# apache/arrow-rs

Measured on NVIDIA B200. Metric: Mrows/sec filter+take+add on 1e9-row Int64/Float64; % HBM roofline, higher is better.
Workload: dtype i64 (filter/take/sum) + f64 (add)

## Files before the change

arrow-rs_b200/csrc/compact.cu:

```cuda
#include <cstdlib>
#include <vector>

#include "bitmap.cuh"
#include "internal.cuh"

#define TILE_ROWS 1024
#define TILE_WORDS (TILE_ROWS / 64)
#define SCAN_CHUNK 4096

struct acu_filter_plan {
  int64_t len = 0;
  int64_t count = 0;
  int32_t strategy = ACU_FILTER_NONE;
  int64_t n_tiles = 0;
  uint64_t *mask = nullptr;
  uint64_t *tile_off = nullptr;
  uint32_t *tile_count = nullptr;
  uint64_t *chunk_total = nullptr;
  void *storage = nullptr;
  mutable void *index_cache = nullptr;
};

namespace {

__global__ void __launch_bounds__(256) k_plan_mask(const uint8_t *__restrict__ pv, int64_t poff,
                                                   const uint8_t *__restrict__ nv, int64_t noff,
                                                   int64_t len, int64_t n_words_padded, uint64_t *__restrict__ mask,
                                                   uint32_t *__restrict__ tile_count, int64_t n_tiles) {
  const int lane = threadIdx.x & 31;
  const int64_t warp = ((int64_t)blockIdx.x * blockDim.x + threadIdx.x) >> 5;
  const int64_t nwarps = ((int64_t)gridDim.x * blockDim.x) >> 5;
  for (int64_t w0 = warp * 32; w0 < n_words_padded; w0 += nwarps * 32) {
    const int64_t w = w0 + lane;
    const int64_t row = w << 6;
    uint64_t m = ld_bits64(pv, poff + row, poff + len);
    if (nv) m &= ld_bits64(nv, noff + row, noff + len);
    mask[w] = m;
    unsigned c = __popcll(m);
#pragma unroll
    for (int o = 8; o > 0; o >>= 1) c += __shfl_xor_sync(ACU_FULL_MASK, c, o);
    const int64_t t = w >> 4;
    if ((lane & 15) == 0 && t < n_tiles) tile_count[t] = c;
  }
}

__global__ void __launch_bounds__(1024) k_plan_scan_chunks(const uint32_t *__restrict__ tile_count, int64_t n_tiles,
                                                           uint64_t *__restrict__ tile_off,
                                                           uint64_t *__restrict__ chunk_total) {
  __shared__ uint32_t warp_tot[32];
  const int64_t base = (int64_t)blockIdx.x * SCAN_CHUNK + (int64_t)threadIdx.x * 4;
  uint32_t c[4];
#pragma unroll
  for (int k = 0; k < 4; ++k) c[k] = (base + k < n_tiles) ? tile_count[base + k] : 0u;
  uint32_t mine = c[0] + c[1] + c[2] + c[3];
  uint32_t incl = mine;
  const int lane = threadIdx.x & 31, wid = threadIdx.x >> 5;
#pragma unroll
  for (int o = 1; o < 32; o <<= 1) {
    uint32_t y = __shfl_up_sync(ACU_FULL_MASK, incl, o);
    if (lane >= o) incl += y;
  }
  if (lane == 31) warp_tot[wid] = incl;
  __syncthreads();
  if (wid == 0) {
    uint32_t w = warp_tot[lane], wi = w;
#pragma unroll
    for (int o = 1; o < 32; o <<= 1) {
      uint32_t y = __shfl_up_sync(ACU_FULL_MASK, wi, o);
      if (lane >= o) wi += y;
    }
    warp_tot[lane] = wi - w;
    if (lane == 31) chunk_total[blockIdx.x] = wi;
  }
  __syncthreads();
  uint32_t excl = warp_tot[wid] + incl - mine;
#pragma unroll
  for (int k = 0; k < 4; ++k) {
    if (base + k < n_tiles) tile_off[base + k] = excl;
    excl += c[k];
  }
}

__global__ void __launch_bounds__(1024) k_plan_scan_top(uint64_t *__restrict__ chunk_total, int64_t n_chunks,
                                                        unsigned long long *__restrict__ res) {
  __shared__ uint64_t warp_tot[32];
  __shared__ uint64_t carry_s;
  if (threadIdx.x == 0) carry_s = 0;
  __syncthreads();
  const int lane = threadIdx.x & 31, wid = threadIdx.x >> 5;
  for (int64_t base = 0; base < n_chunks; base += 1024) {
    const int64_t i = base + threadIdx.x;
    uint64_t v = i < n_chunks ? chunk_total[i] : 0ull, incl = v;
#pragma unroll
    for (int o = 1; o < 32; o <<= 1) {
      uint64_t y = __shfl_up_sync(ACU_FULL_MASK, incl, o);
      if (lane >= o) incl += y;
    }
    if (lane == 31) warp_tot[wid] = incl;
    __syncthreads();
    if (wid == 0) {
      uint64_t w = warp_tot[lane], wi = w;
#pragma unroll
      for (int o = 1; o < 32; o <<= 1) {
        uint64_t y = __shfl_up_sync(ACU_FULL_MASK, wi, o);
        if (lane >= o) wi += y;
      }
      warp_tot[lane] = wi - w;
    }
    __syncthreads();
    const uint64_t carry = carry_s;
    if (i < n_chunks) chunk_total[i] = carry + warp_tot[wid] + incl - v;
    __syncthreads();
    if (threadIdx.x == 1023) carry_s = carry + warp_tot[31] + incl;
    __syncthreads();
  }
  if (threadIdx.x == 0) res[RES_COUNT] = carry_s;
}

__global__ void __launch_bounds__(256) k_plan_finalize(uint64_t *__restrict__ tile_off, int64_t n_tiles, int64_t n_padded,
                                                       const uint64_t *__restrict__ chunk_off,
                                                       const unsigned long long *__restrict__ res) {
  const int64_t stride = (int64_t)gridDim.x * blockDim.x;
  for (int64_t t = (int64_t)blockIdx.x * blockDim.x + threadIdx.x; t < n_padded; t += stride)
    tile_off[t] = t < n_tiles ? tile_off[t] + chunk_off[t / SCAN_CHUNK] : res[RES_COUNT];
}

struct FilterArgs {
  const uint8_t *values;
  uint8_t *out;
  const uint64_t *mask;
  const uint64_t *tile_off;
  int64_t n_tiles;
  int aligned16;
  const uint8_t *vsrc;
  int64_t voff;
  int64_t vlen;
  uint32_t *vout;
  unsigned long long *res;
};

constexpr int BATCH_COLS = 8;
struct FilterBatch { FilterArgs col[BATCH_COLS]; };

template <int W>
__global__ void __launch_bounds__(256, 4) k_filter_values(const FilterBatch batch) {
  const FilterArgs &a = batch.col[blockIdx.y];
  constexpr int CPT = TILE_ROWS * W / 16;
  constexpr int ITERS = CPT / 32;
  constexpr int BATCH = ITERS < 8 ? ITERS : 8;
  constexpr int RPC = W <= 16 ? 16 / W : 1;
  constexpr int CPR = W <= 16 ? 1 : W / 16;
  const int lane = threadIdx.x & 31;
  const int64_t warp = ((int64_t)blockIdx.x * blockDim.x + threadIdx.x) >> 5;
  const int64_t nwarps = ((int64_t)gridDim.x * blockDim.x) >> 5;

  int64_t t = warp;
  uint64_t m_next = 0, off_next = 0, end_next = 0;
  if (t < a.n_tiles) {
    if (lane < TILE_WORDS) m_next = __ldg(a.mask + t * TILE_WORDS + lane);
    off_next = __ldg(a.tile_off + t);
    end_next = __ldg(a.tile_off + t + 1);
  }
  for (; t < a.n_tiles; t += nwarps) {
    const uint64_t m = m_next, out0 = off_next, cnt = end_next - off_next;
    const int64_t tn = t + nwarps;
    if (tn < a.n_tiles) {
      m_next = (lane < TILE_WORDS) ? __ldg(a.mask + tn * TILE_WORDS + lane) : 0ull;
      off_next = __ldg(a.tile_off + tn);
      end_next = __ldg(a.tile_off + tn + 1);
    }
    if (cnt == 0) continue;
    const uint32_t c = __popcll(m);
    uint32_t incl = c;
#pragma unroll
    for (int o = 1; o < TILE_WORDS; o <<= 1) {
      uint32_t y = __shfl_up_sync(ACU_FULL_MASK, incl, o);
      if (lane >= o) incl += y;
    }
    const uint32_t pref = incl - c;
    const uint8_t *src = a.values + (size_t)t * TILE_ROWS * W;
    uint8_t *dst = a.out + (size_t)out0 * W;
#pragma unroll 1
    for (int b0 = 0; b0 < ITERS; b0 += BATCH) {
      uint4 v[BATCH];
      uint32_t bits[BATCH];
      uint32_t rank[BATCH];
#pragma unroll
      for (int j = 0; j < BATCH; ++j) {
        const int cidx = (b0 + j) * 32 + lane;
        const int r = cidx * RPC / CPR;
        const uint64_t word = __shfl_sync(ACU_FULL_MASK, m, r >> 6);
        const uint32_t wp = __shfl_sync(ACU_FULL_MASK, pref, r >> 6);
        bits[j] = (uint32_t)(word >> (r & 63)) & ((1u << RPC) - 1u);
        rank[j] = wp + __popcll(word & ((1ull << (r & 63)) - 1ull));
        if (bits[j]) {
          if (a.aligned16) {
            v[j] = ld_stream16(src + (size_t)cidx * 16);
          } else {
            if constexpr (W >= 8) {
              const uint64_t *p = reinterpret_cast<const uint64_t *>(src + (size_t)cidx * 16);
              const uint64_t lo = (W > 8 || (bits[j] & 1u)) ? __ldg(p) : 0ull;
              const uint64_t hi = (W > 8 || (bits[j] & 2u)) ? __ldg(p + 1) : 0ull;
              v[j] = make_uint4((uint32_t)lo, (uint32_t)(lo >> 32), (uint32_t)hi, (uint32_t)(hi >> 32));
            } else if constexpr (W == 4) {
              const uint32_t *p = reinterpret_cast<const uint32_t *>(src + (size_t)cidx * 16);
              v[j].x = (bits[j] & 1u) ? __ldg(p) : 0u;
              v[j].y = (bits[j] & 2u) ? __ldg(p + 1) : 0u;
              v[j].z = (bits[j] & 4u) ? __ldg(p + 2) : 0u;
              v[j].w = (bits[j] & 8u) ? __ldg(p + 3) : 0u;
            } else {
              uint8_t *vb = reinterpret_cast<uint8_t *>(&v[j]);
              const uint8_t *p = src + (size_t)cidx * 16;
#pragma unroll
              for (int e = 0; e < 16; ++e) vb[e] = ((bits[j] >> (e / W)) & 1u) ? __ldg(p + e) : (uint8_t)0;
// ... 224 lines not shown
    __syncwarp();
    const uint8_t *src = a.values + (size_t)t * TILE_ROWS * W;
    uint8_t *dst = a.out + (size_t)out0 * W;
#pragma unroll 1
    for (int pass = 0; pass < C::PASSES; ++pass) {
      const int half_base = (pass * C::PASS_ROWS) >> 5;
      const uint8_t *psrc = src + ((size_t)pass * C::CPP + lane) * 16;
      asm volatile("" : "+l"(psrc));
      const uint32_t *hh = &s_h[wid][half_base + lr_half];
      uint32_t sel = 0;
#pragma unroll
      for (int j = 0; j < C::ITERS; ++j) {
        const int r0 = j * RPJ;
        const uint32_t bits = (hh[r0 >> 5] >> ((r0 & 31) + lr_bit)) & F::CHUNK_MASK;
        sel |= bits << (j * RPC);
        if (bits) cp_async16(lbuf + j * 32, psrc + (size_t)j * 512);
      }
      cp_async_wait_all();
      __syncwarp();
      const uint32_t *hp = &s_hp[wid][half_base + lr_half];
#pragma unroll
      for (int j = 0; j < C::ITERS; ++j) {
        const uint32_t bits = (sel >> (j * RPC)) & F::CHUNK_MASK;
        const int r0 = j * RPJ;
        const int sh = (r0 & 31) + lr_bit;
        const uint32_t rank = hp[r0 >> 5] + __popc(hh[r0 >> 5] & ((1u << sh) - 1u));
        const uint4 x = lbuf[j * 32];
        if constexpr (W == 8) {
          uint64_t *o = reinterpret_cast<uint64_t *>(dst) + rank;
          if (bits & 1u) o[0] = (uint64_t)x.x | ((uint64_t)x.y << 32);
          if (bits & 2u) o[bits & 1u] = (uint64_t)x.z | ((uint64_t)x.w << 32);
        } else if constexpr (W == 4) {
          uint32_t *o = reinterpret_cast<uint32_t *>(dst) + rank;
          if (bits & 1u) *o++ = x.x;
          if (bits & 2u) *o++ = x.y;
          if (bits & 4u) *o++ = x.z;
          if (bits & 8u) *o = x.w;
        } else if constexpr (W == 2) {
          uint16_t *o = reinterpret_cast<uint16_t *>(dst) + rank;
          const uint16_t *ve = reinterpret_cast<const uint16_t *>(&x);
#pragma unroll
          for (int e = 0; e < 8; ++e)
            if ((bits >> e) & 1u) *o++ = ve[e];
        } else if constexpr (W == 1) {
          uint8_t *o = dst + rank;
          const uint8_t *ve = reinterpret_cast<const uint8_t *>(&x);
#pragma unroll
          for (int e = 0; e < 16; ++e)
            if ((bits >> e) & 1u) *o++ = ve[e];
        } else {
          if (bits) {
            const int half = lane % CPR;
            uint64_t *o = reinterpret_cast<uint64_t *>(dst + (size_t)rank * W + half * 16);
            o[0] = (uint64_t)x.x | ((uint64_t)x.y << 32);
            o[1] = (uint64_t)x.z | ((uint64_t)x.w << 32);
          }
        }
      }
      __syncwarp();
    }
    if (vsrc) {
      const uint32_t c = __popcll(m);
      if (c) {
        const uint64_t bits = pext64_sparse(v, m, c);
        valid_cnt += __popcll(bits);
        const uint64_t p = out0 + s_hp[wid][(2 * lane) & 31];
        const uint32_t sh = (uint32_t)p & 31u;
        uint32_t *o = a.vout + (p >> 5);
        const uint32_t w0 = (uint32_t)(bits << sh);
        const uint64_t rest = sh ? (bits >> (32u - sh)) : (bits >> 32);
        if (w0) atomicOr(o, w0);
        if ((uint32_t)rest) atomicOr(o + 1, (uint32_t)rest);
        if ((uint32_t)(rest >> 32)) atomicOr(o + 2, (uint32_t)(rest >> 32));
      }
      __syncwarp();
    }
  }
  if (vsrc && a.res) {
    valid_cnt = warp_sum(valid_cnt);
    if (lane == 0 && valid_cnt) atomicAdd(a.res + RES_COUNT, (unsigned long long)valid_cnt);
  }
}

struct CompressArgs {
  const uint8_t *src;
  int64_t soff;
  uint32_t *out;
  unsigned long long *res;
  uint64_t out_bytes;
  const uint64_t *count_ptr;
};
struct CompressBatch { CompressArgs col[BATCH_COLS]; };

__global__ void __launch_bounds__(256) k_zero_outputs(const CompressBatch batch) {
  const CompressArgs &c = batch.col[blockIdx.y];
  uint64_t *o = reinterpret_cast<uint64_t *>(c.out);
  const uint64_t words = c.count_ptr ? ((*c.count_ptr + 63) >> 6) : (c.out_bytes >> 3);
  for (uint64_t i = (uint64_t)blockIdx.x * blockDim.x + threadIdx.x; i < words; i += (uint64_t)gridDim.x * blockDim.x) o[i] = 0ull;
}
__global__ void __launch_bounds__(256) k_zero_bitmap_dev(uint64_t *__restrict__ o, const uint64_t *__restrict__ count_ptr) {
  const uint64_t words = (*count_ptr + 63) >> 6;
  for (uint64_t i = (uint64_t)blockIdx.x * blockDim.x + threadIdx.x; i < words; i += (uint64_t)gridDim.x * blockDim.x) o[i] = 0ull;
}

__global__ void __launch_bounds__(256, 8) k_compress_bits(const CompressBatch batch, int64_t len, const uint64_t *__restrict__ mask,
                                                       const uint64_t *__restrict__ tile_off, int64_t n_words_padded) {
  const uint8_t *__restrict__ src = batch.col[blockIdx.y].src;
  const int64_t soff = batch.col[blockIdx.y].soff;
  uint32_t *__restrict__ out = batch.col[blockIdx.y].out;
  unsigned long long *__restrict__ res = batch.col[blockIdx.y].res;
  __shared__ uint32_t s_win[8][68];
  const int lane = threadIdx.x & 31, wid = threadIdx.x >> 5;
  const int64_t warp = ((int64_t)blockIdx.x * blockDim.x + threadIdx.x) >> 5;
  const int64_t nwarps = ((int64_t)gridDim.x * blockDim.x) >> 5;
  unsigned valid_cnt = 0;
  for (int64_t w0 = warp * 32; w0 < n_words_padded; w0 += nwarps * 32) {
    const int64_t w = w0 + lane;
    uint64_t m = __ldg(mask + w);
    const uint32_t cnt = __popcll(m);
    uint32_t incl = cnt;
#pragma unroll
    for (int o = 1; o < 32; o <<= 1) {
      uint32_t y = __shfl_up_sync(ACU_FULL_MASK, incl, o);
      if (lane >= o) incl += y;
    }
    const uint32_t total = __shfl_sync(ACU_FULL_MASK, incl, 31);
    if (total == 0) continue;
    const uint64_t base = __ldg(tile_off + (w0 >> 4));
    uint64_t bits = 0;
    if (m) {
      const uint64_t v = ld_bits64(src, soff + (w << 6), soff + len);
      const uint64_t ones = m & v, zeros = m & ~v;
      const bool clear_mode = __popcll(zeros) <= __popcll(ones);
      uint64_t it = clear_mode ? zeros : ones, acc = 0;
      while (it) {
        const int b = __ffsll((long long)it) - 1;
        it &= it - 1;
        acc |= 1ull << __popcll(m & ((1ull << b) - 1ull));
      }
      const uint64_t full = cnt == 64 ? ~0ull : ((1ull << cnt) - 1ull);
      bits = clear_mode ? (full & ~acc) : acc;
    }
    valid_cnt += __popcll(bits);
    const uint32_t lead = (uint32_t)(base & 31);
    const uint32_t nwords = (lead + total + 31) >> 5;
    for (uint32_t i = lane; i < nwords; i += 32) s_win[wid][i] = 0;
    __syncwarp();
    if (cnt) {
      const uint32_t p = lead + incl - cnt;
      const uint32_t sh = p & 31;
      atomicOr(&s_win[wid][p >> 5], (uint32_t)(bits << sh));
      if (sh + cnt > 32) {
        const uint64_t rest = bits >> (32 - sh);
        atomicOr(&s_win[wid][(p >> 5) + 1], (uint32_t)rest);
        if (sh + cnt > 64) atomicOr(&s_win[wid][(p >> 5) + 2], (uint32_t)(rest >> 32));
      }
    }
    __syncwarp();
    uint32_t *o = out + (base >> 5);
    for (uint32_t i = lane; i < nwords; i += 32) {
      const uint32_t word = s_win[wid][i];
      if (i == 0 || i == nwords - 1) { if (word) atomicOr(o + i, word); }
      else o[i] = word;
    }
    __syncwarp();
  }
  if (res) {
    valid_cnt = warp_sum(valid_cnt);
    if (lane == 0 && valid_cnt) atomicAdd(res + RES_COUNT, (unsigned long long)valid_cnt);
  }
}

acu_status check_len(acu_ctx *ctx, const acu_filter_plan *plan, int64_t values_len) {
  if (plan->len > values_len)
    return acu_fail(ctx, ACU_ERR_INVALID_ARGUMENT, -1, 0, 0, (uint64_t)values_len,
                    "Filter predicate of length %lld is larger than target array of length %lld",
                    (long long)plan->len, (long long)values_len);
  return ACU_OK;
}

template <int W>
acu_status launch_filter(acu_ctx *ctx, const FilterBatch &fb, int n_cols, bool fused) {
  const FilterArgs &fa = fb.col[0];
  if (fa.aligned16) {
    if (!fused) {
      constexpr size_t smem = 8 * (size_t)AsyncCfg<W>::PASS_BYTES;
      if (ctx->occupancy.find(reinterpret_cast<const void *>(k_filter_values_async<W>)) == ctx->occupancy.end())
        ACU_CUDA(ctx, cudaFuncSetAttribute(k_filter_values_async<W>, cudaFuncAttributeMaxDynamicSharedMemorySize, (int)smem));
      const int gx = acu_wave_grid(ctx, k_filter_values_async<W>, 256, smem, (fa.n_tiles + 7) / 8);
      ACU_LAUNCH_TIMED(ctx, ACU_K_FILTER, (k_filter_values_async<W>), dim3(gx, n_cols), 256, smem, fb);
      return ACU_OK;
    }
    constexpr size_t smem = 8 * (size_t)AsyncCfg<W>::PASS_BYTES;
    if (ctx->occupancy.find(reinterpret_cast<const void *>(k_filter_fused<W>)) == ctx->occupancy.end())
      ACU_CUDA(ctx, cudaFuncSetAttribute(k_filter_fused<W>, cudaFuncAttributeMaxDynamicSharedMemorySize, (int)smem));
    static const int tiles_per_warp = getenv("ACU_FILTER_TILES_PER_WARP") ? atoi(getenv("ACU_FILTER_TILES_PER_WARP")) : 4;
    const int64_t want = (fa.n_tiles + 8 * (int64_t)tiles_per_warp - 1) / (8 * (int64_t)tiles_per_warp);
    int gx = acu_wave_grid(ctx, k_filter_fused<W>, 256, smem, (fa.n_tiles + 7) / 8);
    gx = (gx + n_cols - 1) / n_cols;
    if (gx > want) gx = (int)(want < 1 ? 1 : want);
    ACU_LAUNCH_TIMED(ctx, ACU_K_FILTER, (k_filter_fused<W>), dim3(gx, n_cols), 256, smem, fb);
  } else {
    const int gx = acu_wave_grid(ctx, k_filter_values<W>, 256, 0, (fa.n_tiles + 7) / 8);
    ACU_LAUNCH_TIMED(ctx, ACU_K_FILTER, (k_filter_values<W>), dim3(gx, n_cols), 256, 0, fb);
  }
  return ACU_OK;
}

acu_status launch_filter_width(acu_ctx *ctx, int32_t elem_bytes, const FilterBatch &fb, int n_cols, bool fused) {
  switch (elem_bytes) {
    case 1: return launch_filter<1>(ctx, fb, n_cols, fused);
    case 2: return launch_filter<2>(ctx, fb, n_cols, fused);
    case 4: return launch_filter<4>(ctx, fb, n_cols, fused);
    case 8: return launch_filter<8>(ctx, fb, n_cols, fused);
    case 16: return launch_filter<16>(ctx, fb, n_cols, fused);
    case 32: return launch_filter<32>(ctx, fb, n_cols, fused);
    default:
      return acu_fail(ctx, ACU_ERR_INVALID_ARGUMENT, -1, 0, 0, 0, "filter: unsupported element width %d", elem_bytes);
  }
}

acu_status launch_compress(acu_ctx *ctx, const acu_filter_plan *plan, const CompressBatch &cb, int n_cols) {
  const int64_t n_words_padded = ((plan->n_tiles * TILE_WORDS + 31) / 32) * 32;
  const int64_t words = (int64_t)acu_bitmap_bytes(plan->count < 0 ? plan->len : plan->count) / 8;
  ACU_LAUNCH(ctx, k_zero_outputs, dim3(acu_grid(ctx, (words + 255) / 256, 4), n_cols), 256, 0, cb);
  const int gx = acu_wave_grid(ctx, k_compress_bits, 256, 0, (n_words_padded / 32 + 7) / 8);
  ACU_LAUNCH_TIMED(ctx, ACU_K_FILTER, k_compress_bits, dim3(gx, n_cols), 256, 0, cb, plan->len, plan->mask, plan->tile_off, n_words_padded);
  return ACU_OK;
}

CompressArgs compress_args(const acu_filter_plan *plan, const uint8_t *src, int64_t soff, void *out, unsigned long long *res) {
  CompressArgs c;
  c.src = src;
  c.soff = soff;
  c.out = static_cast<uint32_t *>(out);
  c.res = res;
  c.out_bytes = acu_bitmap_bytes(plan->count < 0 ? plan->len : plan->count);
  c.count_ptr = plan->count < 0 ? plan->tile_off + plan->n_tiles : nullptr;
  return c;
}

bool plan_uses_fused(const acu_filter_plan *plan) {
  static const bool legacy = getenv("ACU_FILTER_LEGACY") != nullptr;
  return !legacy && (plan->count < 0 || plan->count * 25 >= plan->len);
}
bool fuses_validity(const acu_filter_plan *plan, const acu_array *values) {
  return plan_uses_fused(plan) && ((uintptr_t)values->values % 16) == 0;
}

FilterArgs filter_args(const acu_filter_plan *plan, const acu_array *values, acu_array_out *out, bool has_nulls,
                       unsigned long long *res) {
  FilterArgs fa{};
  fa.values = static_cast<const uint8_t *>(values->values);
  fa.out = static_cast<uint8_t *>(out->values);
  fa.mask = plan->mask;
  fa.tile_off = plan->tile_off;
  fa.n_tiles = plan->n_tiles;
  fa.aligned16 = ((uintptr_t)values->values % 16) == 0;
  if (has_nulls && fuses_validity(plan, values)) {
    fa.vsrc = values->validity;
    fa.voff = values->validity_offset;
    fa.vlen = plan->len;
    fa.vout = reinterpret_cast<uint32_t *>(out->validity);
    fa.res = res;
  }
  return fa;
}

}

extern "C" {

static acu_status plan_alloc(acu_ctx *ctx, int64_t len, acu_filter_plan **out_plan) {
  acu_filter_plan *plan = new acu_filter_plan();
  plan->len = len;
  *out_plan = plan;
  if (len == 0) return ACU_OK;
  const int64_t n_tiles = (len + TILE_ROWS - 1) / TILE_ROWS;
  const int64_t n_chunks = (n_tiles + SCAN_CHUNK - 1) / SCAN_CHUNK;
  const int64_t n_words_padded = ((n_tiles * TILE_WORDS + 31) / 32) * 32;
  const int64_t n_off_padded = n_words_padded / TILE_WORDS + 2;
  plan->n_tiles = n_tiles;
  auto up = [](size_t x) { return (x + 255) & ~(size_t)255; };
  const size_t mask_b = up((size_t)n_words_padded * 8), off_b = up((size_t)n_off_padded * 8),
               cnt_b = up((size_t)n_tiles * 4), ch_b = up((size_t)n_chunks * 8);
  void *mem = nullptr;
  acu_status st = acu_malloc(ctx, mask_b + off_b + cnt_b + ch_b, &mem);
  if (st != ACU_OK) { delete plan; *out_plan = nullptr; return st; }
  uint8_t *p = static_cast<uint8_t *>(mem);
  plan->storage = mem;
  plan->mask = reinterpret_cast<uint64_t *>(p);
  plan->tile_off = reinterpret_cast<uint64_t *>(p + mask_b);
  plan->tile_count = reinterpret_cast<uint32_t *>(p + mask_b + off_b);
  plan->chunk_total = reinterpret_cast<uint64_t *>(p + mask_b + off_b + cnt_b);
  return ACU_OK;
}

static acu_status plan_finish(acu_ctx *ctx, acu_filter_plan *plan, int kslot, int blk) {
  const int64_t len = plan->len, n_tiles = plan->n_tiles;
  const int64_t n_chunks = (n_tiles + SCAN_CHUNK - 1) / SCAN_CHUNK;
  const int64_t n_words_padded = ((n_tiles * TILE_WORDS + 31) / 32) * 32;
  const int64_t n_off_padded = n_words_padded / TILE_WORDS + 2;
  unsigned long long *res = acu_dres(ctx, blk);
  k_plan_scan_chunks<<<(unsigned)n_chunks, 1024, 0, ctx->stream>>>(plan->tile_count, n_tiles, plan->tile_off, plan->chunk_total);
  k_plan_scan_top<<<1, 1024, 0, ctx->stream>>>(plan->chunk_total, n_chunks, res);
  k_plan_finalize<<<acu_grid(ctx, (n_off_padded + 255) / 256, 8), 256, 0, ctx->stream>>>(plan->tile_off, n_tiles, n_off_padded,
                                                                                     plan->chunk_total, res);
  if (kslot >= 0) acu_kstats_end(ctx, kslot);
  ctx->launches += 3;
  cudaError_t e = cudaGetLastError();
  if (e != cudaSuccess) return acu_cuda_fail(ctx, e, "filter plan kernels");
  plan->count = -1;
  plan->strategy = ACU_FILTER_INDEX;
  return acu_call_end(ctx, blk, [plan, len](const unsigned long long *h) -> acu_status {
    plan->count = (int64_t)h[RES_COUNT];
    if (plan->count == 0) plan->strategy = ACU_FILTER_NONE;
    else if (plan->count == len) plan->strategy = ACU_FILTER_ALL;
    else if ((double)plan->count / (double)len > 0.8) plan->strategy = ACU_FILTER_SLICES;
    else plan->strategy = ACU_FILTER_INDEX;
    return ACU_OK;
  });
}

acu_status acu_filter_plan_create(acu_ctx *ctx, const acu_array *pred, acu_filter_plan **out_plan) {
  *out_plan = nullptr;
  ACU_ENTER(ctx);
  const int64_t len = pred->len;
  acu_status st = ACU_OK;
  int64_t nc = 0;
  if (len > 0) {
    nc = acu_resolve_null_count(ctx, pred, &st);
    ACU_TRY(st);
  }
  acu_filter_plan *plan = nullptr;
  ACU_TRY(plan_alloc(ctx, len, &plan));
  if (len == 0) { *out_plan = plan; return ACU_OK; }
  auto bail = [&](acu_status s) { acu_free(ctx, plan->storage); delete plan; return s; };
  const int64_t n_words_padded = ((plan->n_tiles * TILE_WORDS + 31) / 32) * 32;
  const uint8_t *nv = (pred->validity && nc > 0) ? pred->validity : nullptr;
  const int blk = acu_call_begin(ctx, &st);
  if (st != ACU_OK) return bail(st);
  const int slot = acu_kstats_begin(ctx, ACU_K_FILTER_PLAN);
  k_plan_mask<<<acu_grid(ctx, (n_words_padded / 32 + 7) / 8, 8), 256, 0, ctx->stream>>>(
      static_cast<const uint8_t *>(pred->values), pred->values_offset, nv, pred->validity_offset, len, n_words_padded,
      plan->mask, plan->tile_count, plan->n_tiles);
  ctx->launches += 1;
  st = plan_finish(ctx, plan, slot, blk);
  if (st != ACU_OK) return bail(st);
  *out_plan = plan;
  return ACU_OK;
}

acu_status acu_filter_plan_create_cmp(acu_ctx *ctx, acu_dtype dtype, acu_cmp_op op, const acu_array *a, const acu_array *b,
                                      acu_filter_plan **out_plan) {
  *out_plan = nullptr;
  ACU_ENTER(ctx);
  int64_t len = 0;
  ACU_TRY(acu_cmp_result_len(ctx, a, b, &len));
  acu_filter_plan *plan = nullptr;
  ACU_TRY(plan_alloc(ctx, len, &plan));
  if (len == 0) { *out_plan = plan; return ACU_OK; }
  auto bail = [&](acu_status s) { acu_free(ctx, plan->storage); delete plan; return s; };
  const int64_t n_words_padded = ((plan->n_tiles * TILE_WORDS + 31) / 32) * 32;
  acu_status st = ACU_OK;
  const int blk = acu_call_begin(ctx, &st);
  if (st != ACU_OK) return bail(st);
  st = acu_cmp_into_plan(ctx, dtype, op, a, b, plan->mask, n_words_padded, plan->tile_count, plan->n_tiles);
  if (st != ACU_OK) return bail(st);
  st = plan_finish(ctx, plan, -1, blk);
  if (st != ACU_OK) return bail(st);
  *out_plan = plan;
  return ACU_OK;
}

void acu_filter_plan_destroy(acu_ctx *ctx, acu_filter_plan *plan) {
  if (!plan) return;
  if (plan->storage) acu_free(ctx, plan->storage);
  if (plan->index_cache) acu_free(ctx, plan->index_cache);
  delete plan;
}
int64_t acu_filter_plan_count(const acu_filter_plan *plan) { return plan->count; }
int64_t acu_filter_plan_len(const acu_filter_plan *plan) { return plan->len; }
int32_t acu_filter_plan_strategy(const acu_filter_plan *plan) { return plan->strategy; }

acu_status acu_filter_primitive(acu_ctx *ctx, const acu_filter_plan *plan, int32_t elem_bytes,
                                const acu_array *values, acu_array_out *out) {
  ACU_ENTER(ctx);
  int mode = 0;
  acu_status st = ACU_OK;
  const int blk = acu_call_begin(ctx, &st);
  ACU_TRY(st);
  ACU_TRY(acu_filter_col_launch(ctx, plan, 0, elem_bytes, values, out, acu_dres(ctx, blk), &mode));
  return acu_call_end(ctx, blk, [plan, mode, out](const unsigned long long *h) -> acu_status {
    acu_filter_col_finalize(plan, nullptr, mode, h, out);
    return ACU_OK;
  });
}

acu_status acu_filter_boolean(acu_ctx *ctx, const acu_filter_plan *plan, const acu_array *values,
                              acu_array_out *out) {
  ACU_ENTER(ctx);
  int mode = 0;
  acu_status st = ACU_OK;
  const int blk = acu_call_begin(ctx, &st);
  ACU_TRY(st);
  ACU_TRY(acu_filter_col_launch(ctx, plan, 1, 0, values, out, acu_dres(ctx, blk), &mode));
  return acu_call_end(ctx, blk, [plan, mode, out](const unsigned long long *h) -> acu_status {
    acu_filter_col_finalize(plan, nullptr, mode, h, out);
    return ACU_OK;
  });
}

}

acu_status acu_filter_col_launch(acu_ctx *ctx, const acu_filter_plan *plan, int kind, int32_t elem_bytes,
                                 const acu_array *values, acu_array_out *out, unsigned long long *res, int *mode) {
  *mode = 0;
  ACU_TRY(check_len(ctx, plan, values->len));
  out->len = plan->count;
  out->has_validity = 0;
  out->null_count = 0;
  const bool pending = plan->count < 0;
  if (!pending && (plan->strategy == ACU_FILTER_NONE || plan->count == 0)) return ACU_OK;
  const bool has_nulls = values->validity != nullptr && (values->null_count != 0 || pending);
  if (plan->strategy == ACU_FILTER_ALL) {
    if (kind == 0)
      ACU_CUDA(ctx, cudaMemcpyAsync(out->values, values->values, (size_t)plan->count * elem_bytes, cudaMemcpyDeviceToDevice, ctx->stream));
    else if (kind == 1)
      ACU_TRY(acu_bitmap_and_launch(ctx, static_cast<const uint8_t *>(values->values), values->values_offset, nullptr, 0,
                                    plan->count, static_cast<uint64_t *>(out->values), false));
    if (values->validity) {
      ACU_TRY(acu_bitmap_and_launch(ctx, values->validity, values->validity_offset, nullptr, 0, plan->count,
                                    reinterpret_cast<uint64_t *>(out->validity), true, res));
      *mode = 2;
    }
    return ACU_OK;
  }
  bool fused = false;
  if (kind == 0) {
    FilterBatch fb{};
    fb.col[0] = filter_args(plan, values, out, has_nulls, res);
    fused = fb.col[0].vsrc != nullptr;
    if (fused) {
      if (pending)
        ACU_LAUNCH(ctx, k_zero_bitmap_dev, acu_grid(ctx, (plan->len / 64 + 255) / 256, 2), 256, 0, reinterpret_cast<uint64_t *>(out->validity),
                   plan->tile_off + plan->n_tiles);
      else
        ACU_CUDA(ctx, cudaMemsetAsync(out->validity, 0, acu_bitmap_bytes(plan->count), ctx->stream));
      *mode = pending ? 3 : 1;
    }
    ACU_TRY(launch_filter_width(ctx, elem_bytes, fb, 1, plan_uses_fused(plan)));
  }
  CompressBatch cb{};
  int nc = 0;
  if (kind == 1)
    cb.col[nc++] = compress_args(plan, static_cast<const uint8_t *>(values->values), values->values_offset, out->values, nullptr);
  if (has_nulls && !fused) {
    cb.col[nc++] = compress_args(plan, values->validity, values->validity_offset, out->validity, res);
    *mode = pending ? 3 : 1;
  }
  if (nc) ACU_TRY(launch_compress(ctx, plan, cb, nc));
  return ACU_OK;
}

acu_status acu_filter_cols_launch(acu_ctx *ctx, const acu_filter_plan *plan, int n, const int *kinds, const int32_t *widths,
                                  const acu_array *const *values, acu_array_out *const *outs, unsigned long long *const *res, int *modes) {
  for (int c = 0; c < n; ++c) {
    modes[c] = 0;
    ACU_TRY(check_len(ctx, plan, values[c]->len));
    outs[c]->len = plan->count;
    outs[c]->has_validity = 0;
    outs[c]->null_count = 0;
  }
  if (plan->strategy == ACU_FILTER_NONE || plan->count == 0) return ACU_OK;
  if (plan->strategy == ACU_FILTER_ALL) {
    for (int c = 0; c < n; ++c) ACU_TRY(acu_filter_col_launch(ctx, plan, kinds[c], widths[c], values[c], outs[c], res[c], &modes[c]));
    return ACU_OK;
  }
  std::vector<char> done(n, 0);
  for (int c = 0; c < n; ++c) {
    if (kinds[c] != 0 || done[c]) continue;
    FilterBatch fb{};
    int k = 0;
    const int al = ((uintptr_t)values[c]->values % 16) == 0;
    for (int d = c; d < n && k < BATCH_COLS; ++d) {
      if (kinds[d] != 0 || done[d] || widths[d] != widths[c] || (((uintptr_t)values[d]->values % 16) == 0) != al) continue;
      const bool has_nulls = values[d]->validity != nullptr && values[d]->null_count != 0;
      fb.col[k] = filter_args(plan, values[d], outs[d], has_nulls, res[d]);
      if (fb.col[k].vsrc) {
        ACU_CUDA(ctx, cudaMemsetAsync(outs[d]->validity, 0, acu_bitmap_bytes(plan->count), ctx->stream));
        modes[d] = 1;
      }
      ++k;
      done[d] = 1;
    }
    ACU_TRY(launch_filter_width(ctx, widths[c], fb, k, plan_uses_fused(plan)));
  }
  CompressBatch cb{};
  int k = 0;
  auto flush = [&]() -> acu_status {
    if (k) ACU_TRY(launch_compress(ctx, plan, cb, k));
    k = 0;
    return ACU_OK;
  };
  for (int c = 0; c < n; ++c) {
    if (kinds[c] == 1) {
      cb.col[k++] = compress_args(plan, static_cast<const uint8_t *>(values[c]->values), values[c]->values_offset, outs[c]->values, nullptr);
      if (k == BATCH_COLS) ACU_TRY(flush());
    }
    if (values[c]->validity != nullptr && values[c]->null_count != 0 && !(kinds[c] == 0 && fuses_validity(plan, values[c]))) {
      cb.col[k++] = compress_args(plan, values[c]->validity, values[c]->validity_offset, outs[c]->validity, res[c]);
      modes[c] = 1;
      if (k == BATCH_COLS) ACU_TRY(flush());
    }
  }
  return flush();
}

void acu_filter_col_finalize(const acu_filter_plan *plan, const acu_array *values, int mode,
                             const unsigned long long *hres, acu_array_out *out) {
  (void)values;
  out->len = plan->count;
  out->has_validity = 0;
  out->null_count = 0;
  if (mode == 1) {
    const int64_t null_count = plan->count - (int64_t)hres[RES_COUNT];
    if (null_count > 0) { out->has_validity = 1; out->null_count = null_count; }
  } else if (mode == 3) {
    const int64_t null_count = plan->count - (int64_t)hres[RES_COUNT];
    if (null_count > 0 || (plan->count == plan->len && plan->count > 0)) { out->has_validity = 1; out->null_count = null_count; }
  } else if (mode == 2) {
    out->has_validity = 1;
    out->null_count = plan->count - (int64_t)hres[RES_COUNT];
  }
}

acu_status acu_filter_nulls_internal(acu_ctx *ctx, const acu_filter_plan *plan, const acu_array *a,
                                     acu_array_out *out) {
  int mode = 0;
  ACU_TRY(acu_res_reset(ctx));
  ACU_TRY(acu_filter_col_launch(ctx, plan, 2, 0, a, out, acu_dres(ctx, 0), &mode));
  ACU_TRY(acu_res_fetch(ctx));
  acu_filter_col_finalize(plan, a, mode, acu_hres(ctx, 0), out);
  return ACU_OK;
}

const uint64_t *acu_plan_mask(const acu_filter_plan *p) { return p->mask; }
const uint64_t *acu_plan_tile_off(const acu_filter_plan *p) { return p->tile_off; }
int64_t acu_plan_n_tiles(const acu_filter_plan *p) { return p->n_tiles; }
void **acu_plan_index_cache(const acu_filter_plan *p) { return &p->index_cache; }
int64_t acu_plan_n_words_padded(const acu_filter_plan *p) { return ((p->n_tiles * TILE_WORDS + 31) / 32) * 32; }
```

arrow-rs_b200/csrc/reduce.cu:

```cuda
#include <limits>
#include <type_traits>

#include "bitmap.cuh"
#include "internal.cuh"

namespace {

template <class T> struct KeyOf { using type = T; };
template <> struct KeyOf<double> { using type = int64_t; };
template <> struct KeyOf<float> { using type = int32_t; };

template <class T> __device__ __forceinline__ typename KeyOf<T>::type to_key(T v) {
  if constexpr (std::is_floating_point<T>::value) return total_key(v);
  else return v;
}
template <class T> __device__ __forceinline__ T from_key(typename KeyOf<T>::type k) {
  if constexpr (sizeof(T) == 8 && std::is_floating_point<T>::value) return __longlong_as_double(k ^ (int64_t)((uint64_t)(k >> 63) >> 1));
  else if constexpr (std::is_floating_point<T>::value) return __int_as_float(k ^ (int32_t)((uint32_t)(k >> 31) >> 1));
  else return k;
}

template <class T, int OP> struct AccOf { using type = typename std::conditional<OP == ACU_SUM, T, typename KeyOf<T>::type>::type; };

template <class A, int OP> __device__ __forceinline__ A acc_identity() {
  if constexpr (OP == ACU_SUM) return A(0);
  else if constexpr (OP == ACU_MIN) return std::numeric_limits<A>::max();
  else return std::numeric_limits<A>::lowest();
}
template <class A, int OP> __device__ __forceinline__ A acc_merge(A a, A b) {
  if constexpr (OP == ACU_SUM) {
    if constexpr (std::is_same<A, double>::value) return __dadd_rn(a, b);
    else if constexpr (std::is_same<A, float>::value) return __fadd_rn(a, b);
    else return (A)((typename std::make_unsigned<A>::type)a + (typename std::make_unsigned<A>::type)b);
  } else if constexpr (OP == ACU_MIN) {
    return b < a ? b : a;
  } else {
    return b > a ? b : a;
  }
}
template <class T, int OP> __device__ __forceinline__ typename AccOf<T, OP>::type acc_lift(T v) {
  if constexpr (OP == ACU_SUM) return v;
  else return to_key<T>(v);
}

template <class A> __device__ __forceinline__ A shfl_down_any(A v, int o) {
  if constexpr (sizeof(A) == 8) {
    long long x;
    memcpy(&x, &v, 8);
    x = __shfl_down_sync(ACU_FULL_MASK, x, o);
    memcpy(&v, &x, 8);
    return v;
  } else {
    int x = 0;
    memcpy(&x, &v, sizeof(A));
    x = __shfl_down_sync(ACU_FULL_MASK, x, o);
    memcpy(&v, &x, sizeof(A));
    return v;
  }
}

constexpr int REDUCE_BATCH_COLS = 8;
struct ReduceArgs {
  const void *v;
  int64_t n;
  const uint8_t *valid;
  int64_t voff;
  void *partial;
  unsigned long long *res;
};
struct ReduceBatch { ReduceArgs col[REDUCE_BATCH_COLS]; };

template <class T, int OP>
__global__ void __launch_bounds__(256) k_reduce(const ReduceBatch batch) {
  using A = typename AccOf<T, OP>::type;
  const T *__restrict__ v = static_cast<const T *>(batch.col[blockIdx.y].v);
  const int64_t n = batch.col[blockIdx.y].n;
  const uint8_t *__restrict__ valid = batch.col[blockIdx.y].valid;
  const int64_t voff = batch.col[blockIdx.y].voff;
  A *__restrict__ partial = static_cast<A *>(batch.col[blockIdx.y].partial);
  unsigned long long *__restrict__ res = batch.col[blockIdx.y].res;
  unsigned int *__restrict__ ticket = reinterpret_cast<unsigned int *>(res + RES_AUX3);
  constexpr int U = 8;
  __shared__ A s_part[8];
  __shared__ bool s_last;
  const int lane = threadIdx.x & 31, wid = threadIdx.x >> 5;
  const int64_t warp = ((int64_t)blockIdx.x * blockDim.x + threadIdx.x) >> 5;
  const int64_t nwarps = ((int64_t)gridDim.x * blockDim.x) >> 5;
  const int64_t sgroups = (n + 2047) >> 11;
  A acc = acc_identity<A, OP>();
  unsigned valid_cnt = 0;
  for (int64_t sg = warp; sg < sgroups; sg += nwarps) {
    const int64_t sbase = sg << 11;
    const int64_t wrow = sbase + lane * 64;
    const int64_t k = n - wrow;
    uint64_t vw = k >= 64 ? ~0ull : (k <= 0 ? 0ull : ((~0ull) >> (64 - k)));
    if (valid) vw &= ld_bits64(valid, voff + wrow, voff + n);
    valid_cnt += __popcll(vw);
#pragma unroll 1
    for (int s0 = 0; s0 < 32; s0 += U) {
      if (sbase + s0 * 64 >= n) break;
      T x[U][2];
#pragma unroll
      for (int u = 0; u < U; ++u) {
#pragma unroll
        for (int h = 0; h < 2; ++h) {
          const int64_t i = sbase + (s0 + u) * 64 + h * 32 + lane;
          x[u][h] = i < n ? __ldg(v + i) : T();
        }
      }
#pragma unroll
      for (int u = 0; u < U; ++u) {
        const uint64_t w = __shfl_sync(ACU_FULL_MASK, vw, s0 + u);
#pragma unroll
        for (int h = 0; h < 2; ++h)
          if ((w >> (h * 32 + lane)) & 1ull) acc = acc_merge<A, OP>(acc, acc_lift<T, OP>(x[u][h]));
      }
    }
  }
  valid_cnt = warp_sum(valid_cnt);
#pragma unroll
  for (int o = 16; o > 0; o >>= 1) acc = acc_merge<A, OP>(acc, shfl_down_any(acc, o));
  if (lane == 0) {
    s_part[wid] = acc;
    if (valid_cnt) atomicAdd(res + RES_COUNT, (unsigned long long)valid_cnt);
  }
  __syncthreads();
  if (threadIdx.x == 0) {
    A b = s_part[0];
    for (int w = 1; w < 8; ++w) b = acc_merge<A, OP>(b, s_part[w]);
    partial[blockIdx.x] = b;
    __threadfence();
    s_last = (atomicAdd(ticket, 1u) == gridDim.x - 1);
  }
  __syncthreads();
  if (s_last && wid == 0) {
    __threadfence();
    A f = acc_identity<A, OP>();
    for (unsigned i = lane; i < gridDim.x; i += 32) f = acc_merge<A, OP>(f, *(volatile A *)(partial + i));
#pragma unroll
    for (int o = 16; o > 0; o >>= 1) f = acc_merge<A, OP>(f, shfl_down_any(f, o));
    if (lane == 0) {
      T r;
      if constexpr (OP == ACU_SUM) r = f;
      else r = from_key<T>(f);
      unsigned long long bits = 0;
      memcpy(&bits, &r, sizeof(T));
      res[RES_AUX0] = bits;
      *ticket = 0;
    }
  }
}

template <class T, int OP>
acu_status reduce_launch(acu_ctx *ctx, const ReduceBatch &rb, int n_cols, int64_t max_len) {
  using A = typename AccOf<T, OP>::type;
  static_assert(sizeof(A) <= 16, "partials must fit the per-column scratch");
  const int64_t strips = (max_len + 63) >> 6;
  const int grid = acu_wave_grid(ctx, k_reduce<T, OP>, 256, 0, (strips / 32 + 1 + 7) / 8);
  ACU_LAUNCH_TIMED(ctx, ACU_K_REDUCE, (k_reduce<T, OP>), dim3(grid, n_cols), 256, 0, rb);
  return ACU_OK;
}

template <class T>
acu_status reduce_typed(acu_ctx *ctx, acu_agg_op op, const ReduceBatch &rb, int n_cols, int64_t max_len) {
  switch (op) {
    case ACU_SUM: return reduce_launch<T, ACU_SUM>(ctx, rb, n_cols, max_len);
    case ACU_MIN: return reduce_launch<T, ACU_MIN>(ctx, rb, n_cols, max_len);
    default: return reduce_launch<T, ACU_MAX>(ctx, rb, n_cols, max_len);
  }
}

acu_status reduce_dispatch(acu_ctx *ctx, acu_dtype dtype, acu_agg_op op, const ReduceBatch &rb, int n_cols, int64_t max_len) {
  switch (dtype) {
    case ACU_I8: return reduce_typed<int8_t>(ctx, op, rb, n_cols, max_len);
    case ACU_I16: return reduce_typed<int16_t>(ctx, op, rb, n_cols, max_len);
    case ACU_I32: return reduce_typed<int32_t>(ctx, op, rb, n_cols, max_len);
    case ACU_I64: return reduce_typed<int64_t>(ctx, op, rb, n_cols, max_len);
    case ACU_U8: return reduce_typed<uint8_t>(ctx, op, rb, n_cols, max_len);
    case ACU_U16: return reduce_typed<uint16_t>(ctx, op, rb, n_cols, max_len);
    case ACU_U32: return reduce_typed<uint32_t>(ctx, op, rb, n_cols, max_len);
    case ACU_U64: return reduce_typed<uint64_t>(ctx, op, rb, n_cols, max_len);
    case ACU_F32: return reduce_typed<float>(ctx, op, rb, n_cols, max_len);
    case ACU_F64: return reduce_typed<double>(ctx, op, rb, n_cols, max_len);
  }
  return acu_fail(ctx, ACU_ERR_INVALID_ARGUMENT, -1, 0, 0, 0, "aggregate: dtype %d", (int)dtype);
}

ReduceArgs reduce_args(const acu_array *a, int64_t nc, void *scratch, unsigned long long *res) {
  ReduceArgs r;
  r.v = a->values;
  r.n = a->len;
  r.valid = (a->validity && nc != 0) ? a->validity : nullptr;
  r.voff = a->validity_offset;
  r.partial = scratch;
  r.res = res;
  return r;
}

}

size_t acu_reduce_col_scratch(const acu_ctx *ctx) { return (size_t)ctx->sm_count * 8 * 8 * 16 + 4096; }

acu_status acu_reduce_col_launch(acu_ctx *ctx, acu_dtype dtype, acu_agg_op op, const acu_array *a, int64_t nc, void *scratch,
                                 unsigned long long *res, int *launched) {
  *launched = 0;
  if (a->len == 0 || nc == a->len) return ACU_OK;
  ReduceBatch rb{};
  rb.col[0] = reduce_args(a, nc, scratch, res);
  ACU_TRY(reduce_dispatch(ctx, dtype, op, rb, 1, a->len));
  *launched = 1;
  return ACU_OK;
}

acu_status acu_reduce_cols_launch(acu_ctx *ctx, int n, const acu_dtype *dtypes, const acu_agg_op *ops, const acu_array *arrays,
                                  const int64_t *nc, uint8_t *scratch, size_t scratch_per_col, unsigned long long *const *res, int *launched) {
  char done[ACU_MAX_BATCH_COLUMNS] = {0};
  for (int c = 0; c < n; ++c) {
    launched[c] = 0;
    if (arrays[c].len == 0 || nc[c] == arrays[c].len) done[c] = 1;
  }
  for (int c = 0; c < n; ++c) {
    if (done[c]) continue;
    ReduceBatch rb{};
    int k = 0;
    int64_t max_len = 0;
    for (int d = c; d < n && k < REDUCE_BATCH_COLS; ++d) {
      if (done[d] || dtypes[d] != dtypes[c] || ops[d] != ops[c]) continue;
      rb.col[k++] = reduce_args(&arrays[d], nc[d], scratch + scratch_per_col * d, res[d]);
      if (arrays[d].len > max_len) max_len = arrays[d].len;
      done[d] = 1;
      launched[d] = 1;
    }
    ACU_TRY(reduce_dispatch(ctx, dtypes[c], ops[c], rb, k, max_len));
  }
  return ACU_OK;
}

extern "C" acu_status acu_aggregate(acu_ctx *ctx, acu_dtype dtype, acu_agg_op op, const acu_array *a,
                                    uint64_t *out_bits, int64_t *out_valid_count) {
  ACU_ENTER(ctx);
  *out_bits = 0;
  *out_valid_count = 0;
// ... 24 lines not shown
```

Measured before the change: 155,900.

## Add chunked gather filter for sparse 8-byte columns and contiguous reduce partitioning

```diff
diff --git a/arrow-rs_b200/csrc/compact.cu b/arrow-rs_b200/csrc/compact.cu
--- a/arrow-rs_b200/csrc/compact.cu
+++ b/arrow-rs_b200/csrc/compact.cu
@@ -7,6 +7,7 @@
 #define TILE_ROWS 1024
 #define TILE_WORDS (TILE_ROWS / 64)
 #define SCAN_CHUNK 4096
+#define GATHER_CHUNK 256
 
 struct acu_filter_plan {
   int64_t len = 0;
@@ -17,6 +18,7 @@
   uint64_t *tile_off = nullptr;
   uint32_t *tile_count = nullptr;
   uint64_t *chunk_total = nullptr;
+  uint32_t *chunk_tile = nullptr;
   void *storage = nullptr;
   mutable void *index_cache = nullptr;
 };
@@ -119,10 +121,18 @@
 
 __global__ void __launch_bounds__(256) k_plan_finalize(uint64_t *__restrict__ tile_off, int64_t n_tiles, int64_t n_padded,
                                                        const uint64_t *__restrict__ chunk_off,
-                                                       const unsigned long long *__restrict__ res) {
+                                                       const unsigned long long *__restrict__ res,
+                                                       const uint32_t *__restrict__ tile_count, uint32_t *__restrict__ chunk_tile) {
   const int64_t stride = (int64_t)gridDim.x * blockDim.x;
-  for (int64_t t = (int64_t)blockIdx.x * blockDim.x + threadIdx.x; t < n_padded; t += stride)
-    tile_off[t] = t < n_tiles ? tile_off[t] + chunk_off[t / SCAN_CHUNK] : res[RES_COUNT];
+  for (int64_t t = (int64_t)blockIdx.x * blockDim.x + threadIdx.x; t < n_padded; t += stride) {
+    if (t < n_tiles) {
+      const uint64_t off = tile_off[t] + chunk_off[t / SCAN_CHUNK], end = off + tile_count[t];
+      tile_off[t] = off;
+      for (uint64_t c = (off + GATHER_CHUNK - 1) / GATHER_CHUNK; c * GATHER_CHUNK < end; ++c) chunk_tile[c] = (uint32_t)t;
+    } else {
+      tile_off[t] = res[RES_COUNT];
+    }
+  }
 }
 
 struct FilterArgs {
@@ -130,6 +140,7 @@
   uint8_t *out;
   const uint64_t *mask;
   const uint64_t *tile_off;
+  const uint32_t *chunk_tile;
   int64_t n_tiles;
   int aligned16;
   const uint8_t *vsrc;
@@ -520,6 +531,120 @@
   }
 }
 
+constexpr int GATHER_PER_LANE = GATHER_CHUNK / 32;
+
+template <int W>
+__global__ void __launch_bounds__(256, 4) k_filter_gather(const FilterBatch batch) {
+  static_assert(W == 8, "the gather filter moves 8-byte values");
+  const FilterArgs &a = batch.col[blockIdx.y];
+  __shared__ int64_t s_rows[8][GATHER_CHUNK];
+  const int lane = threadIdx.x & 31, wid = threadIdx.x >> 5;
+  const uint32_t lt = (1u << lane) - 1u;
+  const int64_t warp = ((int64_t)blockIdx.x * blockDim.x + threadIdx.x) >> 5;
+  const int64_t nwarps = ((int64_t)gridDim.x * blockDim.x) >> 5;
+  const uint64_t total = __ldg(a.tile_off + a.n_tiles);
+  const int64_t n_chunks = (int64_t)((total + GATHER_CHUNK - 1) / GATHER_CHUNK);
+  const int64_t n_words = a.n_tiles * TILE_WORDS;
+  const uint64_t *__restrict__ src = reinterpret_cast<const uint64_t *>(a.values);
+  uint64_t *__restrict__ dst = reinterpret_cast<uint64_t *>(a.out);
+  int64_t *rows = s_rows[wid];
+  unsigned valid_cnt = 0;
+
+  int64_t w_n = 0;
+  uint64_t pre_n = 0, m0 = 0, m1 = 0;
+  auto fetch_words = [&](int64_t w) {
+    m0 = w + lane < n_words ? __ldg(a.mask + w + lane) : 0ull;
+    m1 = w + 32 + lane < n_words ? __ldg(a.mask + w + 32 + lane) : 0ull;
+  };
+  auto fetch = [&](int64_t t) {
+    w_n = t * TILE_WORDS;
+    pre_n = __ldg(a.tile_off + t);
+    fetch_words(w_n);
+  };
+  int64_t t_ahead = 0;
+  if (warp < n_chunks) fetch(__ldg(a.chunk_tile + warp));
+  if (warp + nwarps < n_chunks) t_ahead = __ldg(a.chunk_tile + warp + nwarps);
+  for (int64_t c = warp; c < n_chunks; c += nwarps) {
+    const uint64_t r0 = (uint64_t)c * GATHER_CHUNK;
+    const uint64_t r1 = r0 + GATHER_CHUNK < total ? r0 + GATHER_CHUNK : total;
+    const int cnt = (int)(r1 - r0);
+    int64_t w = w_n;
+    uint64_t pre = pre_n;
+    for (int q = 0; pre < r1; ++q) {
+      if (q == 2) { fetch_words(w); q = 0; }
+      const uint64_t m = m0;
+      m0 = m1;
+      const uint32_t pc = __popcll(m);
+      uint32_t incl = pc;
+#pragma unroll
+      for (int o = 1; o < 32; o <<= 1) {
+        const uint32_t y = __shfl_up_sync(ACU_FULL_MASK, incl, o);
+        if (lane >= o) incl += y;
+      }
+      const uint64_t lo = pre + incl - pc;
+      const bool need = pc != 0 && lo < r1 && lo + pc > r0;
+      uint32_t todo = __ballot_sync(ACU_FULL_MASK, need);
+      const uint32_t most = __reduce_max_sync(ACU_FULL_MASK, need ? pc : 0u);
+      if (most * 2 > (uint32_t)__popc(todo) * 5) {
+        while (todo) {
+          const int s = __ffs(todo) - 1;
+          todo &= todo - 1;
+          const uint64_t mw = __shfl_sync(ACU_FULL_MASK, m, s);
+          uint64_t rk = __shfl_sync(ACU_FULL_MASK, lo, s);
+          const int64_t row0 = (w + s) << 6;
+#pragma unroll
+          for (int h = 0; h < 2; ++h) {
+            const uint32_t half = (uint32_t)(mw >> (32 * h));
+            const uint64_t r = rk + __popc(half & lt);
+            if (((half >> lane) & 1u) && r >= r0 && r < r1) rows[r - r0] = row0 + 32 * h + lane;
+            rk += __popc(half);
+          }
+        }
+      } else if (need) {
+        uint64_t it = m, r = lo;
+        const int64_t row0 = (w + lane) << 6;
+        while (it) {
+          const int b = __ffsll((long long)it) - 1;
+          it &= it - 1;
+          if (r >= r0 && r < r1) rows[r - r0] = row0 + b;
+          ++r;
+        }
+      }
+      pre += __shfl_sync(ACU_FULL_MASK, incl, 31);
+      w += 32;
+    }
+    __syncwarp();
+    uint64_t v[GATHER_PER_LANE];
+    uint32_t bit[GATHER_PER_LANE];
+#pragma unroll
+    for (int k = 0; k < GATHER_PER_LANE; ++k) {
+      const int j = k * 32 + lane;
+      v[k] = 0ull;
+      bit[k] = 0u;
+      if (j < cnt) {
+        const int64_t row = rows[j];
+        v[k] = __ldg(src + row);
+        if (a.vsrc) bit[k] = ld_bit(a.vsrc, a.voff + row);
+      }
+    }
+    if (c + nwarps < n_chunks) {
+      fetch(t_ahead);
+      if (c + 2 * nwarps < n_chunks) t_ahead = __ldg(a.chunk_tile + c + 2 * nwarps);
+    }
+#pragma unroll
+    for (int k = 0; k < GATHER_PER_LANE; ++k) {
+      const int j = k * 32 + lane;
+      if (j < cnt) dst[r0 + j] = v[k];
+      if (a.vsrc && k * 32 < ((cnt + 63) & ~63)) {
+        const uint32_t word = __ballot_sync(ACU_FULL_MASK, bit[k] != 0u);
+        if (lane == 0) { a.vout[(r0 >> 5) + k] = word; valid_cnt += __popc(word); }
+      }
+    }
+    __syncwarp();
+  }
+  if (a.vsrc && a.res && lane == 0 && valid_cnt) atomicAdd(a.res + RES_COUNT, (unsigned long long)valid_cnt);
+}
+
 struct CompressArgs {
   const uint8_t *src;
   int64_t soff;
@@ -645,6 +770,19 @@
   return ACU_OK;
 }
 
+bool uses_gather(const acu_filter_plan *plan, int32_t elem_bytes, const acu_array *values) {
+  return elem_bytes == 8 && ((uintptr_t)values->values % 8) == 0 && (plan->count < 0 || plan->count * 8 < plan->len);
+}
+
+acu_status launch_gather(acu_ctx *ctx, const acu_filter_plan *plan, const FilterBatch &fb, int n_cols) {
+  const int64_t rows = plan->count < 0 ? plan->len : plan->count;
+  const int64_t chunks = (rows + GATHER_CHUNK - 1) / GATHER_CHUNK;
+  int gx = acu_wave_grid(ctx, k_filter_gather<8>, 256, 0, (chunks + 7) / 8);
+  gx = (gx + n_cols - 1) / n_cols;
+  ACU_LAUNCH_TIMED(ctx, ACU_K_FILTER, (k_filter_gather<8>), dim3(gx, n_cols), 256, 0, fb);
+  return ACU_OK;
+}
+
 acu_status launch_filter_width(acu_ctx *ctx, int32_t elem_bytes, const FilterBatch &fb, int n_cols, bool fused) {
   switch (elem_bytes) {
     case 1: return launch_filter<1>(ctx, fb, n_cols, fused);
@@ -682,20 +820,21 @@
   static const bool legacy = getenv("ACU_FILTER_LEGACY") != nullptr;
   return !legacy && (plan->count < 0 || plan->count * 25 >= plan->len);
 }
-bool fuses_validity(const acu_filter_plan *plan, const acu_array *values) {
-  return plan_uses_fused(plan) && ((uintptr_t)values->values % 16) == 0;
-}
-
-FilterArgs filter_args(const acu_filter_plan *plan, const acu_array *values, acu_array_out *out, bool has_nulls,
-                       unsigned long long *res) {
+bool fuses_validity(const acu_filter_plan *plan, int32_t elem_bytes, const acu_array *values) {
+  return uses_gather(plan, elem_bytes, values) || (plan_uses_fused(plan) && ((uintptr_t)values->values % 16) == 0);
+}
+
+FilterArgs filter_args(const acu_filter_plan *plan, int32_t elem_bytes, const acu_array *values, acu_array_out *out,
+                       bool has_nulls, unsigned long long *res) {
   FilterArgs fa{};
   fa.values = static_cast<const uint8_t *>(values->values);
   fa.out = static_cast<uint8_t *>(out->values);
   fa.mask = plan->mask;
   fa.tile_off = plan->tile_off;
+  fa.chunk_tile = plan->chunk_tile;
   fa.n_tiles = plan->n_tiles;
   fa.aligned16 = ((uintptr_t)values->values % 16) == 0;
-  if (has_nulls && fuses_validity(plan, values)) {
+  if (has_nulls && fuses_validity(plan, elem_bytes, values)) {
     fa.vsrc = values->validity;
     fa.voff = values->validity_offset;
     fa.vlen = plan->len;
@@ -721,9 +860,9 @@
   plan->n_tiles = n_tiles;
   auto up = [](size_t x) { return (x + 255) & ~(size_t)255; };
   const size_t mask_b = up((size_t)n_words_padded * 8), off_b = up((size_t)n_off_padded * 8),
-               cnt_b = up((size_t)n_tiles * 4), ch_b = up((size_t)n_chunks * 8);
+               cnt_b = up((size_t)n_tiles * 4), ch_b = up((size_t)n_chunks * 8), ct_b = up((size_t)(len / GATHER_CHUNK + 1) * 4);
   void *mem = nullptr;
-  acu_status st = acu_malloc(ctx, mask_b + off_b + cnt_b + ch_b, &mem);
+  acu_status st = acu_malloc(ctx, mask_b + off_b + cnt_b + ch_b + ct_b, &mem);
   if (st != ACU_OK) { delete plan; *out_plan = nullptr; return st; }
   uint8_t *p = static_cast<uint8_t *>(mem);
   plan->storage = mem;
@@ -731,6 +870,7 @@
   plan->tile_off = reinterpret_cast<uint64_t *>(p + mask_b);
   plan->tile_count = reinterpret_cast<uint32_t *>(p + mask_b + off_b);
   plan->chunk_total = reinterpret_cast<uint64_t *>(p + mask_b + off_b + cnt_b);
+  plan->chunk_tile = reinterpret_cast<uint32_t *>(p + mask_b + off_b + cnt_b + ch_b);
   return ACU_OK;
 }
 
@@ -743,7 +883,8 @@
   k_plan_scan_chunks<<<(unsigned)n_chunks, 1024, 0, ctx->stream>>>(plan->tile_count, n_tiles, plan->tile_off, plan->chunk_total);
   k_plan_scan_top<<<1, 1024, 0, ctx->stream>>>(plan->chunk_total, n_chunks, res);
   k_plan_finalize<<<acu_grid(ctx, (n_off_padded + 255) / 256, 8), 256, 0, ctx->stream>>>(plan->tile_off, n_tiles, n_off_padded,
-                                                                                     plan->chunk_total, res);
+                                                                                     plan->chunk_total, res, plan->tile_count,
+                                                                                     plan->chunk_tile);
   if (kslot >= 0) acu_kstats_end(ctx, kslot);
   ctx->launches += 3;
   cudaError_t e = cudaGetLastError();
@@ -877,17 +1018,21 @@
   bool fused = false;
   if (kind == 0) {
     FilterBatch fb{};
-    fb.col[0] = filter_args(plan, values, out, has_nulls, res);
+    fb.col[0] = filter_args(plan, elem_bytes, values, out, has_nulls, res);
     fused = fb.col[0].vsrc != nullptr;
-    if (fused) {
-      if (pending)
-        ACU_LAUNCH(ctx, k_zero_bitmap_dev, acu_grid(ctx, (plan->len / 64 + 255) / 256, 2), 256, 0, reinterpret_cast<uint64_t *>(out->validity),
-                   plan->tile_off + plan->n_tiles);
-      else
-        ACU_CUDA(ctx, cudaMemsetAsync(out->validity, 0, acu_bitmap_bytes(plan->count), ctx->stream));
-      *mode = pending ? 3 : 1;
-    }
-    ACU_TRY(launch_filter_width(ctx, elem_bytes, fb, 1, plan_uses_fused(plan)));
+    if (fused) *mode = pending ? 3 : 1;
+    if (uses_gather(plan, elem_bytes, values)) {
+      ACU_TRY(launch_gather(ctx, plan, fb, 1));
+    } else {
+      if (fused) {
+        if (pending)
+          ACU_LAUNCH(ctx, k_zero_bitmap_dev, acu_grid(ctx, (plan->len / 64 + 255) / 256, 2), 256, 0, reinterpret_cast<uint64_t *>(out->validity),
+                     plan->tile_off + plan->n_tiles);
+        else
+          ACU_CUDA(ctx, cudaMemsetAsync(out->validity, 0, acu_bitmap_bytes(plan->count), ctx->stream));
+      }
+      ACU_TRY(launch_filter_width(ctx, elem_bytes, fb, 1, plan_uses_fused(plan)));
+    }
   }
   CompressBatch cb{};
   int nc = 0;
@@ -916,23 +1061,25 @@
     return ACU_OK;
   }
   std::vector<char> done(n, 0);
+  auto kernel_class = [&](int c) { return uses_gather(plan, widths[c], values[c]) ? 2 : (int)(((uintptr_t)values[c]->values % 16) == 0); };
   for (int c = 0; c < n; ++c) {
     if (kinds[c] != 0 || done[c]) continue;
     FilterBatch fb{};
     int k = 0;
-    const int al = ((uintptr_t)values[c]->values % 16) == 0;
+    const int kc = kernel_class(c);
     for (int d = c; d < n && k < BATCH_COLS; ++d) {
-      if (kinds[d] != 0 || done[d] || widths[d] != widths[c] || (((uintptr_t)values[d]->values % 16) == 0) != al) continue;
+      if (kinds[d] != 0 || done[d] || widths[d] != widths[c] || kernel_class(d) != kc) continue;
       const bool has_nulls = values[d]->validity != nullptr && values[d]->null_count != 0;
-      fb.col[k] = filter_args(plan, values[d], outs[d], has_nulls, res[d]);
+      fb.col[k] = filter_args(plan, widths[d], values[d], outs[d], has_nulls, res[d]);
       if (fb.col[k].vsrc) {
-        ACU_CUDA(ctx, cudaMemsetAsync(outs[d]->validity, 0, acu_bitmap_bytes(plan->count), ctx->stream));
+        if (kc != 2) ACU_CUDA(ctx, cudaMemsetAsync(outs[d]->validity, 0, acu_bitmap_bytes(plan->count), ctx->stream));
         modes[d] = 1;
       }
       ++k;
       done[d] = 1;
     }
-    ACU_TRY(launch_filter_width(ctx, widths[c], fb, k, plan_uses_fused(plan)));
+    if (kc == 2) ACU_TRY(launch_gather(ctx, plan, fb, k));
+    else ACU_TRY(launch_filter_width(ctx, widths[c], fb, k, plan_uses_fused(plan)));
   }
   CompressBatch cb{};
   int k = 0;
@@ -946,7 +1093,7 @@
       cb.col[k++] = compress_args(plan, static_cast<const uint8_t *>(values[c]->values), values[c]->values_offset, outs[c]->values, nullptr);
       if (k == BATCH_COLS) ACU_TRY(flush());
     }
-    if (values[c]->validity != nullptr && values[c]->null_count != 0 && !(kinds[c] == 0 && fuses_validity(plan, values[c]))) {
+    if (values[c]->validity != nullptr && values[c]->null_count != 0 && !(kinds[c] == 0 && fuses_validity(plan, widths[c], values[c]))) {
       cb.col[k++] = compress_args(plan, values[c]->validity, values[c]->validity_offset, outs[c]->validity, res[c]);
       modes[c] = 1;
       if (k == BATCH_COLS) ACU_TRY(flush());
diff --git a/arrow-rs_b200/csrc/reduce.cu b/arrow-rs_b200/csrc/reduce.cu
--- a/arrow-rs_b200/csrc/reduce.cu
+++ b/arrow-rs_b200/csrc/reduce.cu
@@ -1,3 +1,5 @@
+#include <algorithm>
+#include <cstdint>
 #include <limits>
 #include <type_traits>
 
@@ -71,7 +73,7 @@
 struct ReduceBatch { ReduceArgs col[REDUCE_BATCH_COLS]; };
 
 template <class T, int OP>
-__global__ void __launch_bounds__(256) k_reduce(const ReduceBatch batch) {
+__global__ void __launch_bounds__(256, 4) k_reduce(const ReduceBatch batch) {
   using A = typename AccOf<T, OP>::type;
   const T *__restrict__ v = static_cast<const T *>(batch.col[blockIdx.y].v);
   const int64_t n = batch.col[blockIdx.y].n;
@@ -86,26 +88,25 @@
   const int lane = threadIdx.x & 31, wid = threadIdx.x >> 5;
   const int64_t warp = ((int64_t)blockIdx.x * blockDim.x + threadIdx.x) >> 5;
   const int64_t nwarps = ((int64_t)gridDim.x * blockDim.x) >> 5;
-  const int64_t sgroups = (n + 2047) >> 11;
+  const int64_t strips = (n + 63) >> 6;
+  const int64_t row_end = min(n, (strips * (warp + 1) / nwarps) << 6);
   A acc = acc_identity<A, OP>();
   unsigned valid_cnt = 0;
-  for (int64_t sg = warp; sg < sgroups; sg += nwarps) {
-    const int64_t sbase = sg << 11;
+  for (int64_t sbase = (strips * warp / nwarps) << 6; sbase < row_end; sbase += 2048) {
     const int64_t wrow = sbase + lane * 64;
-    const int64_t k = n - wrow;
-    uint64_t vw = k >= 64 ? ~0ull : (k <= 0 ? 0ull : ((~0ull) >> (64 - k)));
-    if (valid) vw &= ld_bits64(valid, voff + wrow, voff + n);
+    const int64_t k = row_end - wrow;
+    uint64_t vw = k <= 0 ? 0ull : (k >= 64 ? ~0ull : ((~0ull) >> (64 - k)));
+    if (valid && vw) vw &= ld_bits64(valid, voff + wrow, voff + row_end);
     valid_cnt += __popcll(vw);
 #pragma unroll 1
-    for (int s0 = 0; s0 < 32; s0 += U) {
-      if (sbase + s0 * 64 >= n) break;
+    for (int s0 = 0; s0 < 32 && sbase + s0 * 64 < row_end; s0 += U) {
       T x[U][2];
 #pragma unroll
       for (int u = 0; u < U; ++u) {
 #pragma unroll
         for (int h = 0; h < 2; ++h) {
           const int64_t i = sbase + (s0 + u) * 64 + h * 32 + lane;
-          x[u][h] = i < n ? __ldg(v + i) : T();
+          x[u][h] = i < row_end ? __ldg(v + i) : T();
         }
       }
 #pragma unroll
@@ -156,8 +157,10 @@
   using A = typename AccOf<T, OP>::type;
   static_assert(sizeof(A) <= 16, "partials must fit the per-column scratch");
   const int64_t strips = (max_len + 63) >> 6;
-  const int grid = acu_wave_grid(ctx, k_reduce<T, OP>, 256, 0, (strips / 32 + 1 + 7) / 8);
-  ACU_LAUNCH_TIMED(ctx, ACU_K_REDUCE, (k_reduce<T, OP>), dim3(grid, n_cols), 256, 0, rb);
+  const int64_t wave = acu_wave_grid(ctx, k_reduce<T, OP>, 256, 0, INT64_MAX) / 8;
+  int64_t grid = wave * std::min<int64_t>(8, std::max<int64_t>(1, strips / (wave * 8 * 32 * 8)));
+  grid = std::min<int64_t>(grid, (strips + 32 * 8 - 1) / (32 * 8));
+  ACU_LAUNCH_TIMED(ctx, ACU_K_REDUCE, (k_reduce<T, OP>), dim3((unsigned)grid, n_cols), 256, 0, rb);
   return ACU_OK;
 }
 
```

After: 157,800, median of 6. +1.2%, better.
